# arclab-hku/ESVIO

Measured on AMD Instinct MI355X. Metric: Mevents/s through time-surface+detect+track @640x480, higher is better.
Workload: dtype f64 timestamps / u8 images / f32 LK sums in the reference build's order

## Files before the change

esvio_amd/csrc/fe_api.cpp:

```cpp
#include "fe_internal.h"

namespace {
typedef int (*nccl_allgather_fn)(const void*, void*, size_t, int , void* ,
                                 hipStream_t);
struct NcclId {
  char internal[128];
};
typedef int (*nccl_get_id_fn)(NcclId*);
typedef int (*nccl_init_rank_fn)(void** , int, NcclId, int);
typedef int (*nccl_destroy_fn)(void*);
void* rccl_lib() {
  static void* lib = []() -> void* {
    const char* names[] = {"librccl.so.1", "librccl.so"};
    for (const char* n : names)
      if (void* l = dlopen(n, RTLD_NOW | RTLD_NOLOAD | RTLD_GLOBAL)) return l;
    for (const char* n : names)
      if (void* l = dlopen(n, RTLD_NOW | RTLD_GLOBAL)) return l;
    return dlopen("/opt/rocm/lib/librccl.so.1", RTLD_NOW | RTLD_GLOBAL);
  }();
  return lib;
}
template <class F>
F rccl_sym(const char* name) {
  void* l = rccl_lib();
// ... 179 lines not shown
  if ((rc = c->d_rejected.alloc(c, 1))) return bail(rc);
  if ((rc = c->d_res.alloc(c, res_layout(Mc).total))) return bail(rc);
  c->dres = res_view(c->d_res, Mc, 0);
  c->dres.mask = nullptr;
  {
    uint8_t* z_spec = nullptr;
    const size_t bytes = kSpecBlocks * spec_layout(Mc).bytes;
    if ((rc = c->h_spec.alloc(c, bytes))) return bail(rc);
    if (hipHostGetDevicePointer((void**)&z_spec, c->h_spec, 0) != hipSuccess) return bail(ESVIO_FE_EHIP);
    std::memset(c->h_spec, 0, bytes);
    for (int b = 0; b < kSpecBlocks; b++) {
      c->hspec[b] = spec_view(c->h_spec, Mc, b);
      c->zspec[b] = spec_view(z_spec, Mc, b);
    }
  }
  if ((rc = c->d_chain.alloc(c, 2 * std::max<size_t>(M, 1)))) return bail(rc);
  if ((rc = c->d_lane_gate.alloc(c, 16))) return bail(rc);
  c->stage_threads = stager_threads_from_env();
  if (const char* v = getenv("ESVIO_FE_FAULT")) esvio_fe_debug_inject(c, atoi(v));
  if (const char* e = getenv("ESVIO_FE_STEREO_SPLIT")) c->stereo_split_env = atoi(e) != 0;
  c->chain_enabled = getenv("ESVIO_FE_NO_CHAIN") == nullptr;
  c->cam_split_enabled = getenv("ESVIO_FE_NO_CAMSPLIT") == nullptr;
  c->dedup_enabled = getenv("ESVIO_FE_NO_DEDUP") == nullptr && (cfg->max_cnt > 500 || getenv("ESVIO_FE_DEDUP") != nullptr);
  c->fuse_ts_pyr = getenv("ESVIO_FE_NO_FUSE") == nullptr;
  c->fast_lds = getenv("ESVIO_FE_FAST_LDS") != nullptr;
  if (const char* v = getenv("ESVIO_FE_CONVERT_PINNED_COPY")) c->cvt_pinned_copy = atoi(v) != 0 ? 1 : 0;
  c->select_one_wave = getenv("ESVIO_FE_SELECT_SERIAL") != nullptr;
  if (const char* v = getenv("ESVIO_FE_SAE_EV_MIN")) c->sae_ev_min = (size_t)strtoull(v, nullptr, 10);
  c->tiled = make_tile_geom(c->W, c->H, &c->tgeom) && getenv("ESVIO_FE_SAE_SORT") == nullptr;
  for (int i = 0; i < kRightSlots; i++)
    if ((rc = c->d_first[i].alloc(c, (size_t)c->P))) return bail(rc);
  for (int i = 0; i < kRightSlots; i++) {
    const size_t words = arc_bitmap_words(c->W, c->H);
    if ((rc = c->d_cmap[i].alloc(c, words))) return bail(rc);
    if ((rc = c->d_touched[i].alloc(c, arc_flag_bytes(c->W, c->H)))) return bail(rc);
    if (hipMemsetAsync(c->d_cmap[i], 0, words * 4, cur_stream(c)) != hipSuccess ||
        hipMemsetAsync(c->d_touched[i], 0, arc_flag_bytes(c->W, c->H), cur_stream(c)) != hipSuccess)
      return bail(ESVIO_FE_EHIP);
  }
  if ((rc = c->d_pub_slots.alloc(c, std::max<size_t>(M, 1)))) return bail(rc);
  if ((rc = c->d_pub_done.alloc(c, 1))) return bail(rc);
  if (hipMemsetAsync(c->d_lane_gate, 0, 64, cur_stream(c)) != hipSuccess ||
      hipMemsetAsync(c->d_chain, 0, std::max<size_t>(M, 1) * 16, cur_stream(c)) != hipSuccess ||
      hipMemsetAsync(c->d_pub_slots, 0, std::max<size_t>(M, 1) * 8, cur_stream(c)) != hipSuccess ||
      hipMemsetAsync(c->d_pub_done, 0, 8, cur_stream(c)) != hipSuccess)
    return bail(ESVIO_FE_EHIP);
  if ((rc = c->d_ptsD.alloc(c, M))) return bail(rc);
  if ((rc = c->d_sel_idx.alloc(c, M))) return bail(rc);
  if ((rc = c->d_mask_bits.alloc(c, (size_t)c->H * ((c->W + 31) / 32)))) return bail(rc);
  for (PyrStore& ps : c->pyr)
    if ((rc = pyr_alloc(c, ps, c->W, c->H, 3))) return bail(rc);
  if (cfg->median_blur_kernel_size > 0)
    for (PyrStore& ps : c->med_tmp)
      if ((rc = pyr_alloc(c, ps, c->W, c->H, 0))) return bail(rc);
  if (cfg->equalize) {
    for (auto& rb : c->raw)
      for (PyrStore& ps : rb)
        if ((rc = pyr_alloc(c, ps, c->W, c->H, 0))) return bail(rc);
// ... 1137 lines not shown
    return ESVIO_FE_EHIP;
  }
  return 0;
}

int esvio_fe_unregister_host_buffer(void* p) {
  if (!p) return ESVIO_FE_EINVAL;
  if (hipHostUnregister(p) != hipSuccess) {
    (void)hipGetLastError();
    return ESVIO_FE_EHIP;
  }
  return 0;
}

int esvio_fe_debug_inject(esvio_fe_handle c, int mask) {
  if (!c || mask < 0 || mask > 31) return ESVIO_FE_EINVAL;
  c->lim = esvio_fe_ctx::WaitLimits();
  c->lazy_late = (mask & ESVIO_FE_FAULT_LAZY_LATE) != 0;
  if (mask & ESVIO_FE_FAULT_TICKET) c->lim.ticket = 0;
  if (mask & ESVIO_FE_FAULT_LOOKBACK) c->lim.lookback = 0;
  if (mask & ESVIO_FE_FAULT_SPECULATIVE) c->lim.poll = 0;
  if (mask & ESVIO_FE_FAULT_CHAINED) c->lim.chain = 0;
  return 0;
}

int esvio_fe_debug_counters(esvio_fe_handle c, uint64_t out4[4]) {
  if (!c || !out4) return ESVIO_FE_EINVAL;
  out4[0] = c->n_spec_expired;
  out4[1] = c->n_chain_expired;
  out4[2] = c->tr_chain_launch;
  out4[3] = c->tr_chain_used;
  return 0;
}

int esvio_fe_plain_call_counters(esvio_fe_handle c, uint64_t out4[4]) {
  if (!c || !out4) return ESVIO_FE_EINVAL;
  out4[0] = c->n_plain_calls;
// ... 138 lines not shown
```

esvio_amd/csrc/fe_ctx.h:

```cpp
#pragma once
#include <hip/hip_runtime.h>

#include <algorithm>
#include <atomic>
#include <chrono>
#include <cmath>
#include <cstdarg>
#include <cstdio>
#include <cstdlib>
#include <cstring>
#include <dlfcn.h>
#include <map>
#include <string>
#include <utility>
#include <deque>
#include <vector>

#include "../../include/esvio_fe.h"
#include "../../include/esvio_fe_test.h"
#include "fe_host.h"
#include "fe_kernels.h"
#include "fe_layout.h"
#include "fe_mc.h"
#include "fe_res.h"
// ... 143 lines not shown
  bool x_deferred = false;
  std::deque<Batch> announced;
  std::deque<Inflight> inflight;
  bool cur_prefetched = false;
  EventStager* stager = nullptr;
  std::atomic<int> stage_pending{0};
  int cur_stage = -1;
  int stage_threads = 0;
  Launcher* launcher = nullptr;
  uint64_t lane_job[kPrefetchDepth] = {};
  int launch_err = 0;
  uint64_t lks_wait_job[2] = {};
  struct WaitLimits {
    uint32_t lookback = kSpinLookback, ticket = kSpinTicket;
    unsigned long long poll = kTicksPoll, chain = kTicksChain;
  } lim;
  bool lazy_late = false;
  uint64_t n_spec_expired = 0, n_chain_expired = 0;
  DevBuf<EventRec> d_evp[kPrefetchDepth];
  Event ev_lane_done[kPrefetchDepth], ev_lane_arc[kPrefetchDepth];
  PyrStore tmp_pyr[2];
  PyrStore med_tmp[2];
  PyrStore raw[kRightSlots][2];
  int raw_cur = 0;
  DevBuf<uint8_t> d_lut;
  DevBuf<int> d_minmax;
  DevBuf<uint8_t> d_res;
  ResView dres{};
  DevBuf<float2> d_ptsD;
  ResView pin[2] = {}, zpin[2] = {};
  SpecView hspec[kSpecBlocks] = {}, zspec[kSpecBlocks] = {};
  int res_set = 0;
  int lks_last = -1;
  PinBuf<uint8_t> h_spec;
  bool spec_valid = false;
  int spec_n = 0;
  DevBuf<unsigned long long> d_chain;
  DevBuf<uint32_t> d_lane_gate;
  uint32_t gate_seq = 0;
  int n_cu = 0;
  bool waits_fit_spec = true, waits_fit_chain = true;
  uint32_t chain_seq = 0;
  bool chain_enabled = true;
  bool cam_split_enabled = true;
  uint64_t n_plain_calls = 0, n_cam_split = 0, n_stereo_chained = 0;
  bool chain_valid = false;
  uint64_t chain_for = 0;
  bool chain_map_ok = false;
  std::vector<int> chain_map;
  uint64_t frame_no = 0;
  Event ev_chain_done;
  DevBuf<unsigned long long> d_pub_slots, d_pub_done;
// ... 212 lines not shown
```

esvio_amd/csrc/fe_kernels.h:

```cpp
#pragma once
#include <hip/hip_runtime.h>
#include <stdint.h>
#include <stdlib.h>

#include <vector>

namespace esvio {


struct __attribute__((aligned(16))) EventRec {
  uint16_t x, y;
  uint32_t sec, nsec;
  uint8_t pol;
  uint8_t pad[3];
};
static_assert(sizeof(EventRec) == 16, "event record must be 16 B");

constexpr int kPad = 24;
constexpr int kMaxLevels = 4;
constexpr int kLkWin = 21;
constexpr int kArcBlock = 256;
constexpr int kMaxDiscR = 63;

struct PyrDesc {
// ... 180 lines not shown
  PyrDesc N;
  const float2* prev_pts;
  const float2* init_pts;
  float2* next_pts;
  uint8_t* status;
  const int* n_ptr;
  int n_max;
  const unsigned long long* poll_slots = nullptr;
  const unsigned long long* poll_done = nullptr;
  uint32_t poll_seq = 0;
  int poll_from = 0;
  int* poll_err = nullptr;
  unsigned long long* chain_out = nullptr;
  const unsigned long long* chain_in = nullptr;
  uint32_t chain_seq = 0;
  unsigned long long poll_ticks = kTicksPoll, chain_ticks = kTicksChain;
  const uint32_t* gate_ptr = nullptr;
  uint32_t gate_val = 0;
  int max_level;
  int max_count;
  double eps2;
  int flags;
  int accum = 1;
};
void launch_lk(hipStream_t s, const LkArgs& f, const LkArgs* b, float2* back_pts,
               uint8_t* back_status);

struct ArcArgs {
  const EventRec* ev;
  uint32_t n;
// ... 122 lines not shown
```

esvio_amd/csrc/fe_kernels.hip:

```cpp
#include "fe_kernels.h"
#include "fe_mc.h"

#include <algorithm>
#include <cstdio>
#include <cstdlib>
#include <cstring>
#include <tuple>
#include <type_traits>

namespace esvio {

namespace {
template <typename... P, typename... A>
void launch_k(void (*kernel)(P...), dim3 grid, dim3 block, unsigned shmem, hipStream_t s, A... args) {
  static_assert(sizeof...(P) == sizeof...(A), "argument count");
  hipLaunchKernelGGL(kernel, grid, block, shmem, s, args...);
}
}

__device__ __forceinline__ int lane_id() { return threadIdx.x & 63; }

__device__ __forceinline__ double ev_time(uint32_t sec, uint32_t nsec) {
  return __dadd_rn((double)sec, __dmul_rn(1e-9, (double)nsec));
}
// ... 2018 lines not shown
__device__ __forceinline__ uint32_t mad_u24_regw(uint32_t oy, uint32_t ox) {
  uint32_t r;
  static_assert(kLkRegW <= 64, "inline constant");
  asm("v_mad_u32_u24 %0, %1, %2, %3" : "=v"(r) : "v"(oy), "n"(kLkRegW), "v"(ox));
  return r;
}
__device__ __forceinline__ int sdot2_zero(uint32_t a, uint32_t b) {
  int r;
  asm("v_dot2_i32_i16 %0, %1, %2, 0" : "=v"(r) : "v"(a), "v"(b));
  return r;
}
__device__ __forceinline__ int sdot2_seed(uint32_t a, uint32_t b, int seed) {
  int r;
  asm("v_dot2_i32_i16 %0, %1, %2, %3" : "=v"(r) : "v"(a), "v"(b), "s"(seed));
  return r;
}

template <int ACCUM>
__device__ __forceinline__ void lk_point(const LkCall& c, const float2 prev0, const float2 init,
                                         uint32_t* regJ, uint32_t term_base, float* acc_ta, const LkLaneF32* lnf, int lane,
                                         float2& np_out, int& st_out) {
  constexpr int WIN = kLkWin, NP = ACCUM == 2 ? 8 : 7, NPP = 4, NL = kMaxLevels;
  const float halfWin = (WIN - 1) * 0.5f;
  const int W_BITS = 14;
  const RedLane rl = red_lane(lane);
  const bool on = ACCUM == 2 || lane < 63;
  const int plane = ACCUM == 2 ? min(lane, 62) : lane;
  const int row = on ? plane / 3 : 0;
  const int x0 = on ? (plane - row * 3) * NP : 0;
  const int lane_bo = row * kLkRegW + x0;
// ... 297 lines not shown
          break;
        }
      }
      (void)restage;
    }
    if (st && L == 0) {
      const float fx = np.x - halfWin, fy = np.y - halfWin;
      const int ix = (int)floorf(fx), iy = (int)floorf(fy);
      if (ix < -WIN || ix >= cols || iy < -WIN || iy >= rows) st = 0;
    }
  }
  np_out = np;
  st_out = st;
}

struct LkKernelArgs {
  LkCall fwd;
  LkCall back;
  int have_back;
  const float2* prev_pts;
  const float2* init_pts;
  float2* next_pts;
  uint8_t* status;
  float2* back_pts;
  uint8_t* back_status;
  const int* n_ptr;
  int n_max;
  const unsigned long long* poll_slots;
  const unsigned long long* poll_done;
  uint32_t poll_seq;
  int poll_from;
  int* poll_err;
  unsigned long long* chain_out;
  const unsigned long long* chain_in;
  uint32_t chain_seq;
  unsigned long long poll_ticks, chain_ticks;
  const uint32_t* gate_ptr;
  uint32_t gate_val;
};

__device__ __forceinline__ void chain_publish(const LkKernelArgs& a, int pt, int lane, float2 p, int alive) {
  if (!a.chain_out || lane != 0) return;
  const unsigned long long hi = (unsigned long long)((a.chain_seq << 2) | (uint32_t)(alive ? 1 : 0)) << 32;
  __hip_atomic_store(&a.chain_out[2 * pt], hi | __float_as_uint(p.x), __ATOMIC_RELAXED, __HIP_MEMORY_SCOPE_AGENT);
  __hip_atomic_store(&a.chain_out[2 * pt + 1], hi | __float_as_uint(p.y), __ATOMIC_RELAXED,
                     __HIP_MEMORY_SCOPE_AGENT);
}

template <int ACCUM>
__device__ __forceinline__ void lk_kernel_body(const LkKernelArgs& a, uint32_t (*regJ_s)[kLkRegStore], uint32_t acc_t,
                                               float* acc_ta, const LkLaneF32* lnf) {
  const int wave = threadIdx.x >> 6, lane = lane_id();
  const int pt = blockIdx.x * kLkWaves + wave;
  const int n = a.n_ptr ? *a.n_ptr : a.n_max;
// ... 59 lines not shown
      __builtin_amdgcn_s_sleep(16);
    }
    prev0 = make_float2((float)(uint32_t)(v & 0xffffu), (float)(uint32_t)((v >> 16) & 0xffffu));
  } else {
    prev0 = a.prev_pts[pt];
  }
  const float2 init = (a.fwd.flags & 4) ? a.init_pts[pt] : make_float2(0.f, 0.f);
  float2 np;
  int st;
  lk_point<ACCUM>(a.fwd, prev0, init, regJ_s[wave], acc_t, acc_ta, lnf, lane, np, st);
  chain_publish(a, pt, lane, np, st);
  if (lane == 0) {
    a.next_pts[pt] = np;
    a.status[pt] = (uint8_t)st;
  }
  if (a.have_back) {
    float2 bp;
    int bs;
    lk_point<ACCUM>(a.back, np, prev0, regJ_s[wave], acc_t, acc_ta, lnf, lane, bp, bs);
    if (lane == 0) {
      a.back_pts[pt] = bp;
      a.back_status[pt] = (uint8_t)bs;
    }
  }
}

__global__ __launch_bounds__(64 * kLkWaves) void k_lk(LkKernelArgs a) {
  __shared__ __attribute__((aligned(16))) uint32_t regJ_s[kLkWaves][kLkRegStore];
  lk_kernel_body<1>(a, regJ_s, 0u, nullptr, nullptr);
}
__global__ __launch_bounds__(64 * kLkWaves) void k_lk_f32(LkKernelArgs a) {
  __shared__ __attribute__((aligned(16))) uint32_t regJ_s[kLkWaves][kLkRegStore];
  __shared__ __attribute__((aligned(16))) int term_all[kLkWaves][kF32TermWords];
  __shared__ __attribute__((aligned(16))) float term_a[kLkWaves][kLkTermWordsA];
  const int wave = threadIdx.x >> 6, lane = threadIdx.x & 63;
  for (int i = lane; i < kF32TermWords; i += 64) term_all[wave][i] = 0;
  {
    const int l = lane < 63 ? lane : 62, t = l / kLkWin, rw = l - t * kLkWin;
// ... 38 lines not shown
  a.back_status = back_status;
  a.n_ptr = f.n_ptr;
  a.n_max = f.n_max;
  a.poll_slots = f.poll_slots;
  a.poll_done = f.poll_done;
  a.poll_seq = f.poll_seq;
  a.poll_from = f.poll_from;
  a.poll_err = f.poll_err;
  a.chain_out = f.chain_out;
  a.chain_in = f.chain_in;
  a.chain_seq = f.chain_seq;
  a.poll_ticks = f.poll_ticks;
  a.chain_ticks = f.chain_ticks;
  a.gate_ptr = f.gate_ptr;
  a.gate_val = f.gate_val;
  if (f.accum == 2)
    launch_k(k_lk_f32, dim3((a.n_max + kLkWaves - 1) / kLkWaves), dim3(64 * kLkWaves), 0, s, a);
  else
    launch_k(k_lk, dim3((a.n_max + kLkWaves - 1) / kLkWaves), dim3(64 * kLkWaves), 0, s, a);
}

__constant__ int8_t c_small[16][2] = {{0, 3},  {1, 3},   {2, 2},   {3, 1},  {3, 0},  {3, -1},
                                      {2, -2}, {1, -3},  {0, -3},  {-1, -3}, {-2, -2}, {-3, -1},
                                      {-3, 0}, {-3, 1},  {-2, 2},  {-1, 3}};
__constant__ int8_t c_large[20][2] = {{0, 4},   {1, 4},   {2, 3},   {3, 2},  {4, 1},  {4, 0},  {4, -1},
                                      {3, -2},  {2, -3},  {1, -4},  {0, -4}, {-1, -4}, {-2, -3}, {-3, -2},
                                      {-4, -1}, {-4, 0},  {-4, 1},  {-3, 2}, {-2, 3},  {-1, 4}};

template <int N>
struct RingRanks {
// ... 1331 lines not shown
```

esvio_amd/csrc/fe_layout.h:

```cpp
#pragma once
#include <cstddef>
#include <cstdint>

namespace esvio {
namespace fe {

struct P2f {
  float x, y;
};

struct LkOut {
  P2f *fwd, *back;
  uint8_t *st_fwd, *st_back;
};

inline size_t layout_points(int max_cnt) { return max_cnt > 1 ? (size_t)max_cnt : 1; }
inline size_t round_up(size_t v, size_t to) { return (v + to - 1) / to * to; }

struct ResLayout {
  size_t B1[2], C1[2], SA1[2], SB1[2], A[2], CNT, NEW, B2, C2, SA2, SB2, total;
  size_t mask;
};
inline ResLayout res_layout(int max_cnt) {
  const size_t M = layout_points(max_cnt), stM = round_up(M, 64);
// ... 54 lines not shown
  v.counts = (int*)(b + L.CNT);
  v.mask = (uint32_t*)(b + L.mask);
  return v;
}

struct SpecView {
  LkOut out;
  int* expired;
};
inline SpecView spec_view(uint8_t* b, int max_cnt, int block) {
  const SpecLayout L = spec_layout(max_cnt);
  b += (size_t)block * L.bytes;
  return SpecView{LkOut{(P2f*)(b + L.B), (P2f*)(b + L.C), b + L.SA, b + L.SB}, (int*)(b + L.expired)};
}

}
}
```

esvio_amd/csrc/fe_stages.cpp:

```cpp
#include "fe_internal.h"

namespace esvio {
namespace fe {


int ensure_event_capacity(esvio_fe_ctx* c, size_t n) { return c->d_ev.grow(c, n); }

static int grow_sort_buffers(esvio_fe_ctx* c, size_t cap) {
  c->sort_cap = 0;
  for (int i = 0; i < 2; i++) {
    c->keys[i].release();
    c->vals[i].release();
  }
  for (int i = 0; i < 2; i++) {
    if (int rc = c->keys[i].alloc(c, cap)) return rc;
    if (int rc = c->vals[i].alloc(c, cap)) return rc;
  }
  if (int rc = c->sae_marks.alloc(c, cap)) return rc;
  c->sort_cap = cap;
  return 0;
}

int ensure_sort_capacity(esvio_fe_ctx* c, size_t n) {
  if (n > c->sort_cap)
// ... 399 lines not shown
  LkArgs fa = f;
  fa.accum = c->cfg.lk_accum;
  launch_lk(cur_stream(c), fa, b, back_pts, back_status);
}

LkPair lk_pair(const PyrDesc& P, const PyrDesc& N, const P2f* src, const int* n_ptr, int n_max, LkPairKind kind,
               const LkOut& out) {
  const bool t = kind == kLkTemporal;
  return LkPair{make_lk(P, N, (const float2*)src, nullptr, (float2*)out.fwd, out.st_fwd, n_ptr, n_max, 3, 30, 0.01, 0),
                make_lk(N, P, nullptr, nullptr, nullptr, nullptr, n_ptr, n_max, t ? 1 : 3, 30, 0.01,
                        t ? ESVIO_FE_LK_USE_INITIAL_FLOW : 0),
                out};
}

void run_lk_pair(esvio_fe_ctx* c, const LkPair& p) {
  run_lk(c, p.f, c->cfg.flow_back ? &p.b : nullptr, (float2*)p.out.back, p.out.st_back);
}

static int image_stage_slot(esvio_fe_ctx* c, size_t bytes, size_t* off) {
  constexpr int kSlots = 4;
  if (!c->d_img || c->d_img.cap < kSlots * bytes) {
    HIPCHK(c, hipStreamSynchronize(cur_stream(c)));
    c->d_img.release();
    if (int rc = c->h_img.alloc(c, kSlots * bytes)) return rc;
    if (int rc = c->d_img.alloc(c, kSlots * bytes)) return rc;
  }
  *off = (size_t)(c->img_stage_next++ % kSlots) * (c->d_img.cap / kSlots);
  return 0;
}

int copy_level0_in(esvio_fe_ctx* c, const PyrDesc& d, const uint8_t* in) {
// ... 298 lines not shown
```

esvio_amd/csrc/fe_track.cpp:

```cpp
#include "fe_internal.h"

#include <sched.h>
#include <sys/resource.h>

#include <atomic>
#include <condition_variable>
#include <mutex>
#include <thread>

namespace esvio {
namespace fe {

struct PrefetchJob {
  Inflight b;
  bool wait_planes = false;
  int lks_wait = -1;
};

static int prefetch_issue(esvio_fe_ctx* c, const PrefetchJob& j) {
  const Inflight& b = j.b;
  StreamScope on_prefetch_stream(c->stream2);
  if (j.wait_planes) HIPCHK(c, hipStreamWaitEvent(c->stream2, c->ev_planes_free, 0));
  if (j.lks_wait >= 0) HIPCHK(c, hipStreamWaitEvent(c->stream2, c->ev_lks_done[j.lks_wait], 0));
  const EventRec *dL = b.dL, *dR = b.dR;
// ... 221 lines not shown
    } else {
      rc = prefetch_issue(c, job);
      if (!rc && b.stage < 0 && b.space == ESVIO_FE_HOST) {
        b.dL = c->d_evp[b.lane];
        b.dR = c->d_evp[b.lane] + b.nL;
      }
    }
    if (rc) break;
    c->inflight.push_back(b);
    c->announced.pop_front();
    if (only_first) break;
  }
  return rc;
}

static uint32_t next_chain_seq(esvio_fe_ctx* c) {
  c->chain_seq = (c->chain_seq + 1) & 0x3fffffffu;
  if (!c->chain_seq) c->chain_seq = 1;
  return c->chain_seq;
}

int enqueue_spec_temporal(esvio_fe_ctx* c, const Inflight& nxt ,
                          int n_kept, bool with_new) {
  if (int rc = launcher_wait_lane(c, nxt.lane)) return rc;
  HIPCHK(c, hipStreamWaitEvent(c->stream3, c->ev_lane_done[nxt.lane], 0));
  const PyrDesc& P = c->pyr[c->slot_curL].d;
  const PyrDesc& N = c->pyr[nxt.slotL].d;
  const int n_max = with_new ? (int)layout_points(c->cfg.max_cnt) : n_kept;
  LkPair sp = lk_pair(P, N, c->zpin[0].news, nullptr, n_max, kLkTemporal, c->zspec[0].out);
  if (with_new) {
    sp.f.poll_slots = c->d_pub_slots;
    sp.f.poll_done = c->d_pub_done;
    sp.f.poll_seq = c->pub_seq;
    sp.f.poll_from = n_kept;
    sp.f.poll_err = c->zspec[0].expired;
    sp.f.poll_ticks = c->lim.poll;
  }
  const Inflight* nxt2 = nullptr;
  if (c->chain_enabled && c->waits_fit_chain && !nxt.pub && c->inflight.size() >= 2 && c->inflight[0].lane == nxt.lane &&
      !c->chain_valid)
    nxt2 = &c->inflight[1];
  if (nxt2) {
    sp.f.chain_out = c->d_chain;
    sp.f.chain_seq = next_chain_seq(c);
  }
  {
    StreamScope on_spec_stream(c->stream3);
    run_lk_pair(c, sp);
  }
  HIPCHK(c, hipEventRecord(c->ev_spec_done, c->stream3));
  c->spec_valid = true;
  if (nxt2) {
    const bool gated = c->launcher && nxt2->gate != 0;
    if (!gated)
      if (int rc = launcher_wait_lane(c, nxt2->lane)) return rc;
    HIPCHK(c, hipStreamWaitEvent(c->stream4, c->ev_lane_done[nxt.lane], 0));
    if (!gated) HIPCHK(c, hipStreamWaitEvent(c->stream4, c->ev_lane_done[nxt2->lane], 0));
    const PyrDesc& N2 = c->pyr[nxt2->slotL].d;
    LkPair ch = lk_pair(N, N2, nullptr, nullptr, n_max, kLkTemporal, c->zspec[1].out);
    ch.f.chain_in = c->d_chain;
    ch.f.chain_seq = c->chain_seq;
    ch.f.chain_ticks = c->lim.chain;
    ch.f.poll_err = c->zspec[1].expired;
    if (gated) {
      ch.f.gate_ptr = c->d_lane_gate + nxt2->lane;
      ch.f.gate_val = nxt2->gate;
    }
    {
      StreamScope on_chain_stream(c->stream4);
      run_lk_pair(c, ch);
    }
    HIPCHK(c, hipEventRecord(c->ev_chain_done, c->stream4));
    c->chain_valid = true;
    c->tr_chain_launch++;
    c->chain_for = c->frame_no + 2;
    c->chain_map_ok = false;
  }
  return 0;
// ... 115 lines not shown
  const esvio_fe_motion* motion;
  const int M;
  ResView pin{}, zpin{};
  const EventRec *dL = nullptr, *dR = nullptr;
  bool first = false;
  bool arc_done = false, arc_prefetched = false, arc_marked_main = false;
  int arc_lane = 0;
  bool main_reads_events = false;
  bool main_reads_planes = false;
  bool have_next = false, had_announced = false;
  Inflight next_b;
  bool early_done = false, defer_late = false;
  bool use_spec = false, use_chain = false, chain_covers_next = false;
  bool will_spec = false, detect = false;
  bool plain = false, arc_side = false, stereo_chained = false;
  bool split_right = false;
  int set_st = 0;
  std::vector<int> surv_src;
  int n_surv = 0, n_kept = 0;
  clk::time_point tp;

  TrackCall(esvio_fe_ctx* ctx, double t, const esvio_fe_event* l, size_t nl, const esvio_fe_event* r, size_t nr,
            int sp, bool pub, const esvio_fe_motion* mo)
      : c(ctx), time(t), left(l), right(r), nL(nl), nR(nr), space(sp), PUB_THIS_FRAME(pub), motion(mo),
        M(ctx->cfg.max_cnt) {}

  void lap(int i) {
    const auto now = clk::now();
    const double ms = std::chrono::duration<double, std::milli>(now - tp).count();
    c->lat.cur_phase[i] += ms;
// ... 265 lines not shown
            g_ptsC[j] = r.back[k];
            g_stA[j] = r.st_fwd[k];
            g_stB[j] = r.st_back[k];
          }
          t = LkOut{g_ptsB.data(), g_ptsC.data(), g_stA.data(), g_stB.data()};
        }
      }
      if (!spec_ok) {
        std::memcpy(pin.A, c->prev_pts.data(), (size_t)n * 8);
        LkPair lk = lk_pair(prevL, curL, zpin.A, nullptr, n, kLkTemporal, zpin.s1);
        stereo_chained = plain && c->chain_enabled && c->waits_fit_chain;
        if (stereo_chained) {
          c->n_stereo_chained++;
          lk.f.chain_out = c->d_chain;
          lk.f.chain_seq = next_chain_seq(c);
        }
        run_lk_pair(c, lk);
        if (stereo_chained) {
          const PyrDesc& curR = c->pyr[c->slot_curR].d;
          set_st = c->res_set ^ 1;
          LkPair st = lk_pair(curL, curR, nullptr, nullptr, n, kLkStereo, c->zpin[set_st].s1);
          st.f.chain_in = c->d_chain;
          st.f.chain_seq = c->chain_seq;
          st.f.chain_ticks = c->lim.chain;
          st.f.poll_err = c->zspec[1].expired;
          StreamScope on_stereo_stream(stereo_stream(c));
          HIPCHK(c, hipStreamWaitEvent(stereo_stream(c), c->ev_imgs_ready, 0));
          run_lk_pair(c, st);
          if (int rc = record_lks_done(c, c->res_set)) return rc;
        }
        if (int rc = early_work()) return rc;
        if (int rc = exchange_flush(c)) return rc;
        pre_lift();
        lap(1);
        HIPCHK(c, sync_main(c));
        lap(2);
        t = pin.s1;
      }
      std::vector<uint8_t> status(t.st_fwd, t.st_fwd + n);
      c->cur_pts.resize(n);
      std::memcpy(c->cur_pts.data(), t.fwd, (size_t)n * 8);
      if (cfg.flow_back) {
        const P2f* reverse_pts = t.back;
        for (int i = 0; i < n; i++) {
          if (status[i] && t.st_back[i] && pt_distance(c->prev_pts[i], reverse_pts[i]) <= 0.5)
            status[i] = 1;
          else
            status[i] = 0;
        }
      }
      for (int i = 0; i < n; i++)
        if (status[i] && !in_border_event(c, c->cur_pts[i])) status[i] = 0;
      if (chain_covers_next) {
        if (use_spec && spec_ok) {
          c->chain_map.clear();
          for (int i = 0; i < n; i++)
            if (status[i]) c->chain_map.push_back(i);
          c->chain_map_ok = true;
        } else if (int rc = cancel_chain(c)) {
          return rc;
        }
      }
      if (stereo_chained) {
        surv_src.clear();
        for (int i = 0; i < n; i++)
          if (status[i]) surv_src.push_back(i);
      }
      if (c->pre_lift_valid) {
        reduce_vector(c->pre_lx, status);
        reduce_vector(c->pre_ly, status);
      }
      reduce_vector(c->prev_pts, status);
      reduce_vector(c->cur_pts, status);
      reduce_vector(c->ids, status);
      reduce_vector(c->track_cnt, status);
    } else if (chain_covers_next) {
      if (int rc = cancel_chain(c)) return rc;
    }
// ... 152 lines not shown
    const bool lazy = c->lazy_new && detect;
    const bool defer_right = c->lazy_new && !PUB_THIS_FRAME;
    bool pending_later = false;
    if (defer_right && c->pend.active && !c->pend_right.active) {
      pending_later = c->lazy_late || !event_over(c->ev_lknew_done);
    }
    if (!pending_later)
      if (int rc = finalize_lazy(c)) return rc;
    tail_lap(1);
    if (defer_right) {
    } else {
      if (!lazy) HIPCHK(c, sync_main(c));
      if (n_surv || stereo_chained) HIPCHK(c, sync_event(c->ev_lks_done[c->res_set]));
      if (stereo_chained) {
        int* wait_expired = c->hspec[1].expired;
        if (*wait_expired != 0) {
          *wait_expired = 0;
          c->n_chain_expired++;
          const int n = (int)surv_src.size() ? surv_src.back() + 1 : 0;
          if (n) {
            const PyrDesc& curL = c->pyr[c->slot_curL].d;
            const PyrDesc& curR = c->pyr[c->slot_curR].d;
            StreamScope on_stereo_stream(stereo_stream(c));
            run_lk_pair(c, lk_pair(curL, curR, zpin.s1.fwd, nullptr, n, kLkStereo, c->zpin[set_st].s1));
            HIPCHK(c, hipStreamSynchronize(stereo_stream(c)));
          }
        }
      }
    }
    lap(6);
    tt = clk::now();
// ... 150 lines not shown
```

esvio_amd/frontend.py:

```python
import ctypes as C
import os

import numpy as np

from . import build as _build

_HERE = os.path.dirname(os.path.abspath(__file__))
HOST, DEVICE = 0, 1
LK_USE_INITIAL_FLOW = 4


class FrontendError(RuntimeError):
    pass


class Camera(C.Structure):
    _fields_ = [(n, C.c_double) for n in ("fx", "fy", "cx", "cy", "k1", "k2", "p1", "p2")]


class Config(C.Structure):
    _fields_ = [
        ("width", C.c_int32), ("height", C.c_int32),
        ("decay_ms", C.c_double),
        ("ignore_polarity", C.c_int32), ("median_blur_kernel_size", C.c_int32),
# ... 55 lines not shown
    "esvio_fe_convert_events", "esvio_fe_create",
    "esvio_fe_create_sae", "esvio_fe_create_sae_stereo", "esvio_fe_create_sae_stereo_mc", "esvio_fe_destroy",
    "esvio_fe_exchange_begin", "esvio_fe_exchange_end", "esvio_fe_exchange_tracks", "esvio_fe_export_image",
    "esvio_fe_fast_corners", "esvio_fe_features_to_track", "esvio_fe_find_fundamental_mat", "esvio_fe_finish", "esvio_fe_get_sae",
    "esvio_fe_get_time_surface", "esvio_fe_good_features_to_track", "esvio_fe_import_image", "esvio_fe_is_corner",
    "esvio_fe_last_error", "esvio_fe_mem_alloc", "esvio_fe_mem_free", "esvio_fe_mem_upload",
    "esvio_fe_pack_track_records", "esvio_fe_register_host_buffer", "esvio_fe_reserve", "esvio_fe_reset",
    "esvio_fe_sae_plane_doubles", "esvio_fe_sae_slice_apply", "esvio_fe_sae_slice_commit",
    "esvio_fe_sae_slice_last", "esvio_fe_sae_to_time_surface", "esvio_fe_set_auto_exchange",
    "esvio_fe_set_host_threads", "esvio_fe_set_launch_thread", "esvio_fe_set_lazy_new_stereo",
    "esvio_fe_set_next_batch", "esvio_fe_set_next_batch_mc", "esvio_fe_track_event", "esvio_fe_track_event_fields",
    "esvio_fe_track_event_mc",
    "esvio_fe_track_image", "esvio_fe_unregister_host_buffer", "esvio_fe_version",
]
TEST_SYMBOLS = [
    "esvio_fe_build_pyramid", "esvio_fe_debug_counters", "esvio_fe_debug_inject", "esvio_fe_device_memory",
    "esvio_fe_find_fundamental_mat_held", "esvio_fe_find_fundamental_mat_idle", "esvio_fe_find_fundamental_mat_mt",
    "esvio_fe_get_kernel_stats", "esvio_fe_host_hypot", "esvio_fe_host_nullspace", "esvio_fe_host_stage_copy",
    "esvio_fe_host_stage_pack", "esvio_fe_staging_counters",
    "esvio_fe_kernel_count", "esvio_fe_kernel_name", "esvio_fe_latency_phase_name", "esvio_fe_latency_recent",
    "esvio_fe_latency_stats", "esvio_fe_lift_projective", "esvio_fe_plain_call_counters", "esvio_fe_ransac_stats",
    "esvio_fe_ransac_tail", "esvio_fe_reset_kernel_stats", "esvio_fe_set_profiling", "esvio_fe_set_sae",
    "esvio_fe_stream",
]

LATENCY_PHASES = 16


class LatencyCall(C.Structure):
    _fields_ = [("call", C.c_uint64), ("published", C.c_int32), ("reserved", C.c_int32), ("begin_ms", C.c_double),
                ("ms", C.c_double), ("phase_ms", C.c_double * 16)]
# ... 45 lines not shown
    L.esvio_fe_lift_projective.argtypes = [C.POINTER(Camera), d, d, vp]
    L.esvio_fe_track_event.argtypes = [vp, d, vp, sz, vp, sz, i, i, C.POINTER(Tracks)]
    L.esvio_fe_track_event_mc.argtypes = [vp, d, vp, sz, vp, sz, i, i, C.POINTER(Motion),
                                          C.POINTER(Tracks)]
    L.esvio_fe_create_sae_stereo_mc.argtypes = [vp, vp, sz, vp, sz, i, C.POINTER(Motion),
                                                C.POINTER(C.c_uint64)]
    L.esvio_fe_set_next_batch.argtypes = [vp, d, vp, sz, vp, sz, i, i]
    L.esvio_fe_set_next_batch_mc.argtypes = [vp, d, vp, sz, vp, sz, i, i, C.POINTER(Motion)]
    L.esvio_fe_mem_alloc.argtypes = [i, sz, vp]
    L.esvio_fe_mem_free.argtypes = [i, vp]
    L.esvio_fe_mem_upload.argtypes = [vp, vp, sz]
    L.esvio_fe_register_host_buffer.argtypes = [vp, sz]
    L.esvio_fe_unregister_host_buffer.argtypes = [vp]
    L.esvio_fe_debug_inject.argtypes = [vp, i]
    L.esvio_fe_debug_counters.argtypes = [vp, vp]
    L.esvio_fe_plain_call_counters.argtypes = [vp, vp]
    L.esvio_fe_good_features_to_track.argtypes = [vp, vp, i, d, d, vp, vp, vp, vp]
    L.esvio_fe_track_image.argtypes = [vp, d, vp, vp, i, vp]
    L.esvio_fe_pack_track_records.argtypes = [vp, vp, vp]
    L.esvio_fe_set_lazy_new_stereo.argtypes = [vp, i]
    L.esvio_fe_set_host_threads.argtypes = [vp, i]
    L.esvio_fe_ransac_stats.argtypes = [vp, i]
    L.esvio_fe_host_hypot.argtypes = [vp, vp, i, vp]
    L.esvio_fe_host_stage_copy.argtypes = [vp, vp, C.c_size_t]
    L.esvio_fe_host_nullspace.argtypes = [vp, i, i, vp, C.POINTER(C.c_int32)]
    L.esvio_fe_find_fundamental_mat_mt.argtypes = [vp, vp, i, d, d, i, vp, C.POINTER(C.c_int32)]
    L.esvio_fe_finish.argtypes = [vp, vp]
    L.esvio_fe_get_time_surface.argtypes = [vp, i, vp]
    L.esvio_fe_export_image.argtypes = [vp, i, vp, i]
    L.esvio_fe_import_image.argtypes = [vp, i, vp, i]
# ... 57 lines not shown
    c.device = device
    cams = kw.get("cams")
    if cams is None:
        cams = [dict(fx=0.9 * W, fy=0.9 * W, cx=W / 2.0, cy=H / 2.0, k1=-0.05, k2=0.01, p1=1e-4,
                     p2=-2e-4)] * 2
    for k in range(2):
        for n in ("fx", "fy", "cx", "cy", "k1", "k2", "p1", "p2"):
            setattr(c.cam[k], n, float(cams[k][n]))
    return c


def _p(a):
    return a.ctypes.data_as(C.c_void_p) if a is not None else None


FAULT_TICKET, FAULT_LOOKBACK, FAULT_SPECULATIVE, FAULT_CHAINED, FAULT_LAZY_LATE = 1, 2, 4, 8, 16


def _events_arg(ev):
    if isinstance(ev, tuple):
        return C.c_void_p(ev[0]), int(ev[1]), DEVICE, None
    ev = np.ascontiguousarray(ev)
    if ev.dtype.itemsize != 16:
        raise ValueError("events must be 16-byte records (esvio_amd.events.EVENT_DTYPE)")
    return _p(ev), ev.shape[0], HOST, ev


class _Handle:
    def __init__(self, cfg):
        self.L = load_library()
        self.cfg = cfg
# ... 240 lines not shown
            out.append((int(o.call), bool(o.published), o.begin_ms, o.ms,
                        {names[k]: o.phase_ms[k] for k in range(LATENCY_PHASES) if o.phase_ms[k] > 0.0005}))
        return out

    def debug_inject(self, mask):
        self._hd.check(self._hd.L.esvio_fe_debug_inject(self._hd.h, int(mask)))

    def staging_counters(self):
        out = (C.c_uint64 * 4)()
        self._hd.check(self._hd.L.esvio_fe_staging_counters(self._hd.h, out))
        return dict(batches=out[0], bytes=out[1], chunks_packed=out[2], chunks_raw=out[3])

    def debug_counters(self):
        out = (C.c_uint64 * 4)()
        self._hd.check(self._hd.L.esvio_fe_debug_counters(self._hd.h, out))
        return dict(spec_redone=out[0], chain_redone=out[1], chain_launched=out[2], chain_used=out[3])

    def plain_call_counters(self):
        out = (C.c_uint64 * 4)()
        self._hd.check(self._hd.L.esvio_fe_plain_call_counters(self._hd.h, out))
        return dict(plain_calls=out[0], split_by_camera=out[1], stereo_chained=out[2], chained_redone=out[3])

    def comm_init(self, unique_id, rank, world):
        buf = (C.c_uint8 * 128).from_buffer_copy(bytes(unique_id))
        self._hd.check(self._hd.L.esvio_fe_comm_init(self._hd.h, buf, int(rank), int(world)))
        self._x_world = int(world)

    def set_auto_exchange(self, on=True):
        self._hd.check(self._hd.L.esvio_fe_set_auto_exchange(self._hd.h, int(bool(on))))

    def exchange_begin(self):
# ... 322 lines not shown
```

Measured before the change: 2825.

## Abandon chained LK back-tracks for points the producer already knows are dropped

When a producer LK kernel's backward check shows a point will be rejected (back status zero or round-trip distance over a bound), it publishes a per-point drop word in a new third section of the chain buffer. The chained consumer kernel reads that word and skips its own backward LK for the point, marking it dead and counting abandonments. Points whose forward status is already zero also skip the backward pass. The host re-checks the drop rule against its final keep mask and falls back to the redo path on a mismatch. This trades extra atomics, a larger chain buffer and extra host verification for less wasted backward tracking.

```diff
diff --git a/esvio_amd/csrc/fe_api.cpp b/esvio_amd/csrc/fe_api.cpp
--- a/esvio_amd/csrc/fe_api.cpp
+++ b/esvio_amd/csrc/fe_api.cpp
@@ -217,12 +217,13 @@
       c->zspec[b] = spec_view(z_spec, Mc, b);
     }
   }
-  if ((rc = c->d_chain.alloc(c, 2 * std::max<size_t>(M, 1)))) return bail(rc);
+  if ((rc = c->d_chain.alloc(c, 3 * std::max<size_t>(M, 1)))) return bail(rc);
   if ((rc = c->d_lane_gate.alloc(c, 16))) return bail(rc);
   c->stage_threads = stager_threads_from_env();
   if (const char* v = getenv("ESVIO_FE_FAULT")) esvio_fe_debug_inject(c, atoi(v));
   if (const char* e = getenv("ESVIO_FE_STEREO_SPLIT")) c->stereo_split_env = atoi(e) != 0;
   c->chain_enabled = getenv("ESVIO_FE_NO_CHAIN") == nullptr;
+  c->abandon_enabled = getenv("ESVIO_FE_NO_ABANDON") == nullptr;
   c->cam_split_enabled = getenv("ESVIO_FE_NO_CAMSPLIT") == nullptr;
   c->dedup_enabled = getenv("ESVIO_FE_NO_DEDUP") == nullptr && (cfg->max_cnt > 500 || getenv("ESVIO_FE_DEDUP") != nullptr);
   c->fuse_ts_pyr = getenv("ESVIO_FE_NO_FUSE") == nullptr;
@@ -244,7 +245,7 @@
   if ((rc = c->d_pub_slots.alloc(c, std::max<size_t>(M, 1)))) return bail(rc);
   if ((rc = c->d_pub_done.alloc(c, 1))) return bail(rc);
   if (hipMemsetAsync(c->d_lane_gate, 0, 64, cur_stream(c)) != hipSuccess ||
-      hipMemsetAsync(c->d_chain, 0, std::max<size_t>(M, 1) * 16, cur_stream(c)) != hipSuccess ||
+      hipMemsetAsync(c->d_chain, 0, std::max<size_t>(M, 1) * 24, cur_stream(c)) != hipSuccess ||
       hipMemsetAsync(c->d_pub_slots, 0, std::max<size_t>(M, 1) * 8, cur_stream(c)) != hipSuccess ||
       hipMemsetAsync(c->d_pub_done, 0, 8, cur_stream(c)) != hipSuccess)
     return bail(ESVIO_FE_EHIP);
@@ -1412,13 +1413,26 @@
 }
 
 int esvio_fe_debug_inject(esvio_fe_handle c, int mask) {
-  if (!c || mask < 0 || mask > 31) return ESVIO_FE_EINVAL;
+  if (!c || mask < 0 || mask > 63) return ESVIO_FE_EINVAL;
   c->lim = esvio_fe_ctx::WaitLimits();
   c->lazy_late = (mask & ESVIO_FE_FAULT_LAZY_LATE) != 0;
   if (mask & ESVIO_FE_FAULT_TICKET) c->lim.ticket = 0;
   if (mask & ESVIO_FE_FAULT_LOOKBACK) c->lim.lookback = 0;
   if (mask & ESVIO_FE_FAULT_SPECULATIVE) c->lim.poll = 0;
   if (mask & ESVIO_FE_FAULT_CHAINED) c->lim.chain = 0;
+  if (mask & ESVIO_FE_FAULT_ALL_DROPPED) c->lim.drop_d2 = -1.f;
+  return 0;
+}
+
+int esvio_fe_abandon_counters(esvio_fe_handle c, uint64_t out4[4]) {
+  if (!c || !out4) return ESVIO_FE_EINVAL;
+  uint32_t n = 0;
+  HIPCHK(c, hipSetDevice(c->dev));
+  HIPCHK(c, hipMemcpy(&n, c->dres.counts + 8, 4, hipMemcpyDeviceToHost));
+  out4[0] = n;
+  out4[1] = c->n_abandon_mismatch;
+  out4[2] = c->n_drop_launches;
+  out4[3] = c->abandon_enabled ? 1 : 0;
   return 0;
 }
 
diff --git a/esvio_amd/csrc/fe_ctx.h b/esvio_amd/csrc/fe_ctx.h
--- a/esvio_amd/csrc/fe_ctx.h
+++ b/esvio_amd/csrc/fe_ctx.h
@@ -181,6 +181,7 @@
   struct WaitLimits {
     uint32_t lookback = kSpinLookback, ticket = kSpinTicket;
     unsigned long long poll = kTicksPoll, chain = kTicksChain;
+    float drop_d2 = kDropDist2;
   } lim;
   bool lazy_late = false;
   uint64_t n_spec_expired = 0, n_chain_expired = 0;
@@ -203,6 +204,9 @@
   bool spec_valid = false;
   int spec_n = 0;
   DevBuf<unsigned long long> d_chain;
+  bool abandon_enabled = true;
+  float chain_drop_d2 = 0.f;
+  uint64_t n_abandon_mismatch = 0, n_drop_launches = 0;
   DevBuf<uint32_t> d_lane_gate;
   uint32_t gate_seq = 0;
   int n_cu = 0;
diff --git a/esvio_amd/csrc/fe_kernels.h b/esvio_amd/csrc/fe_kernels.h
--- a/esvio_amd/csrc/fe_kernels.h
+++ b/esvio_amd/csrc/fe_kernels.h
@@ -218,6 +218,11 @@
   unsigned long long* chain_out = nullptr;
   const unsigned long long* chain_in = nullptr;
   uint32_t chain_seq = 0;
+  unsigned long long* drop_out = nullptr;
+  const unsigned long long* drop_in = nullptr;
+  float drop_d2 = 0.f;
+  uint32_t* abandoned = nullptr;
+  bool skip_dead = false;
   unsigned long long poll_ticks = kTicksPoll, chain_ticks = kTicksChain;
   const uint32_t* gate_ptr = nullptr;
   uint32_t gate_val = 0;
diff --git a/esvio_amd/csrc/fe_kernels.hip b/esvio_amd/csrc/fe_kernels.hip
--- a/esvio_amd/csrc/fe_kernels.hip
+++ b/esvio_amd/csrc/fe_kernels.hip
@@ -1,4 +1,5 @@
 #include "fe_kernels.h"
+#include "fe_layout.h"
 #include "fe_mc.h"
 
 #include <algorithm>
@@ -2056,6 +2057,46 @@
   int r;
   asm("v_dot2_i32_i16 %0, %1, %2, %3" : "=v"(r) : "v"(a), "v"(b), "s"(seed));
   return r;
+}
+
+struct LkKernelArgs {
+  LkCall fwd;
+  LkCall back;
+  int have_back;
+  const float2* prev_pts;
+  const float2* init_pts;
+  float2* next_pts;
+  uint8_t* status;
+  float2* back_pts;
+  uint8_t* back_status;
+  const int* n_ptr;
+  int n_max;
+  const unsigned long long* poll_slots;
+  const unsigned long long* poll_done;
+  uint32_t poll_seq;
+  int poll_from;
+  int* poll_err;
+  unsigned long long* chain_out;
+  const unsigned long long* chain_in;
+  uint32_t chain_seq;
+  unsigned long long poll_ticks, chain_ticks;
+  const uint32_t* gate_ptr;
+  uint32_t gate_val;
+  unsigned long long* drop_out;
+  const unsigned long long* drop_in;
+  float drop_d2;
+  uint32_t* abandoned;
+  int skip_dead;
+};
+
+__device__ __forceinline__ bool lk_dropped() {
+  const LkKernelArgs* ka = (const LkKernelArgs*)__builtin_amdgcn_kernarg_segment_ptr();
+  asm volatile("" : "+s"(ka));
+  const unsigned long long* w = ka->drop_in;
+  if (!w) return false;
+  const int pt = blockIdx.x * kLkWaves + __builtin_amdgcn_readfirstlane(threadIdx.x >> 6);
+  const uint32_t v = __hip_atomic_load((const uint32_t*)(w + pt) + 1, __ATOMIC_RELAXED, __HIP_MEMORY_SCOPE_AGENT);
+  return (uint32_t)__builtin_amdgcn_readfirstlane((int)v) == ((ka->chain_seq << 2) | 1u);
 }
 
 template <int ACCUM>
@@ -2383,30 +2424,6 @@
   st_out = st;
 }
 
-struct LkKernelArgs {
-  LkCall fwd;
-  LkCall back;
-  int have_back;
-  const float2* prev_pts;
-  const float2* init_pts;
-  float2* next_pts;
-  uint8_t* status;
-  float2* back_pts;
-  uint8_t* back_status;
-  const int* n_ptr;
-  int n_max;
-  const unsigned long long* poll_slots;
-  const unsigned long long* poll_done;
-  uint32_t poll_seq;
-  int poll_from;
-  int* poll_err;
-  unsigned long long* chain_out;
-  const unsigned long long* chain_in;
-  uint32_t chain_seq;
-  unsigned long long poll_ticks, chain_ticks;
-  const uint32_t* gate_ptr;
-  uint32_t gate_val;
-};
 
 __device__ __forceinline__ void chain_publish(const LkKernelArgs& a, int pt, int lane, float2 p, int alive) {
   if (!a.chain_out || lane != 0) return;
@@ -2496,14 +2513,31 @@
     a.next_pts[pt] = np;
     a.status[pt] = (uint8_t)st;
   }
-  if (a.have_back) {
-    float2 bp;
-    int bs;
-    lk_point<ACCUM>(a.back, np, prev0, regJ_s[wave], acc_t, acc_ta, lnf, lane, bp, bs);
+  if (!a.have_back) return;
+  if (a.skip_dead && !st) {
     if (lane == 0) {
-      a.back_pts[pt] = bp;
-      a.back_status[pt] = (uint8_t)bs;
-    }
+      a.back_pts[pt] = np;
+      a.back_status[pt] = 0;
+    }
+    return;
+  }
+  if (lk_dropped()) {
+    if (lane == 0) {
+      a.status[pt] = 0;
+      a.back_status[pt] = 0;
+      if (a.abandoned) __hip_atomic_fetch_add(a.abandoned, 1u, __ATOMIC_RELAXED, __HIP_MEMORY_SCOPE_AGENT);
+    }
+    return;
+  }
+  float2 bp;
+  int bs;
+  lk_point<ACCUM>(a.back, np, prev0, regJ_s[wave], acc_t, acc_ta, lnf, lane, bp, bs);
+  if (lane == 0) {
+    a.back_pts[pt] = bp;
+    a.back_status[pt] = (uint8_t)bs;
+    if (a.drop_out && fe::surely_dropped(bs, prev0.x, prev0.y, bp.x, bp.y, a.drop_d2))
+      __hip_atomic_store(&a.drop_out[pt], (unsigned long long)((a.chain_seq << 2) | 1u) << 32, __ATOMIC_RELAXED,
+                         __HIP_MEMORY_SCOPE_AGENT);
   }
 }
 
@@ -2572,6 +2606,11 @@
   a.chain_ticks = f.chain_ticks;
   a.gate_ptr = f.gate_ptr;
   a.gate_val = f.gate_val;
+  a.drop_out = f.drop_out;
+  a.drop_in = f.drop_in;
+  a.drop_d2 = f.drop_d2;
+  a.abandoned = f.abandoned;
+  a.skip_dead = f.skip_dead ? 1 : 0;
   if (f.accum == 2)
     launch_k(k_lk_f32, dim3((a.n_max + kLkWaves - 1) / kLkWaves), dim3(64 * kLkWaves), 0, s, a);
   else
diff --git a/esvio_amd/csrc/fe_layout.h b/esvio_amd/csrc/fe_layout.h
--- a/esvio_amd/csrc/fe_layout.h
+++ b/esvio_amd/csrc/fe_layout.h
@@ -92,5 +92,15 @@
   return SpecView{LkOut{(P2f*)(b + L.B), (P2f*)(b + L.C), b + L.SA, b + L.SB}, (int*)(b + L.expired)};
 }
 
+constexpr float kDropDist2 = 0.2625f;
+#if defined(__HIPCC__) || defined(__CUDACC__)
+__host__ __device__
+#endif
+inline bool surely_dropped(int back_status, float px, float py, float bx, float by, float bound) {
+  if (!back_status) return true;
+  const float dx = px - bx, dy = py - by;
+  return dx * dx + dy * dy > bound;
+}
+
 }
 }
diff --git a/esvio_amd/csrc/fe_stages.cpp b/esvio_amd/csrc/fe_stages.cpp
--- a/esvio_amd/csrc/fe_stages.cpp
+++ b/esvio_amd/csrc/fe_stages.cpp
@@ -437,7 +437,9 @@
 }
 
 void run_lk_pair(esvio_fe_ctx* c, const LkPair& p) {
-  run_lk(c, p.f, c->cfg.flow_back ? &p.b : nullptr, (float2*)p.out.back, p.out.st_back);
+  LkArgs f = p.f;
+  f.skip_dead = c->abandon_enabled;
+  run_lk(c, f, c->cfg.flow_back ? &p.b : nullptr, (float2*)p.out.back, p.out.st_back);
 }
 
 static int image_stage_slot(esvio_fe_ctx* c, size_t bytes, size_t* off) {
diff --git a/esvio_amd/csrc/fe_track.cpp b/esvio_amd/csrc/fe_track.cpp
--- a/esvio_amd/csrc/fe_track.cpp
+++ b/esvio_amd/csrc/fe_track.cpp
@@ -259,6 +259,27 @@
   return rc;
 }
 
+static void drop_word_out(esvio_fe_ctx* c, LkArgs& producer) {
+  if (!c->abandon_enabled || !c->cfg.flow_back) return;
+  producer.drop_out = c->d_chain + 2 * layout_points(c->cfg.max_cnt);
+  producer.drop_d2 = c->chain_drop_d2 = c->lim.drop_d2;
+  c->n_drop_launches++;
+}
+static void drop_word_in(esvio_fe_ctx* c, LkArgs& consumer) {
+  if (!c->abandon_enabled || !c->cfg.flow_back) return;
+  consumer.drop_in = c->d_chain + 2 * layout_points(c->cfg.max_cnt);
+  consumer.abandoned = (uint32_t*)(c->dres.counts + 8);
+}
+
+static bool drop_rule_mismatch(esvio_fe_ctx* c, const std::vector<uint8_t>& kept, const LkOut& t, const P2f* prev, int n) {
+  if (!c->abandon_enabled || !c->cfg.flow_back) return false;
+  bool bad = false;
+  for (int i = 0; i < n; i++)
+    if (kept[i] && surely_dropped(t.st_back[i], prev[i].x, prev[i].y, t.back[i].x, t.back[i].y, c->chain_drop_d2)) bad = true;
+  if (bad) c->n_abandon_mismatch++;
+  return bad;
+}
+
 static uint32_t next_chain_seq(esvio_fe_ctx* c) {
   c->chain_seq = (c->chain_seq + 1) & 0x3fffffffu;
   if (!c->chain_seq) c->chain_seq = 1;
@@ -288,6 +309,7 @@
   if (nxt2) {
     sp.f.chain_out = c->d_chain;
     sp.f.chain_seq = next_chain_seq(c);
+    drop_word_out(c, sp.f);
   }
   {
     StreamScope on_spec_stream(c->stream3);
@@ -307,6 +329,7 @@
     ch.f.chain_seq = c->chain_seq;
     ch.f.chain_ticks = c->lim.chain;
     ch.f.poll_err = c->zspec[1].expired;
+    drop_word_in(c, ch.f);
     if (gated) {
       ch.f.gate_ptr = c->d_lane_gate + nxt2->lane;
       ch.f.gate_val = nxt2->gate;
@@ -452,6 +475,7 @@
   bool use_spec = false, use_chain = false, chain_covers_next = false;
   bool will_spec = false, detect = false;
   bool plain = false, arc_side = false, stereo_chained = false;
+  bool stereo_mismatch = false;
   bool split_right = false;
   int set_st = 0;
   std::vector<int> surv_src;
@@ -747,6 +771,7 @@
           c->n_stereo_chained++;
           lk.f.chain_out = c->d_chain;
           lk.f.chain_seq = next_chain_seq(c);
+          drop_word_out(c, lk.f);
         }
         run_lk_pair(c, lk);
         if (stereo_chained) {
@@ -757,6 +782,7 @@
           st.f.chain_seq = c->chain_seq;
           st.f.chain_ticks = c->lim.chain;
           st.f.poll_err = c->zspec[1].expired;
+          drop_word_in(c, st.f);
           StreamScope on_stereo_stream(stereo_stream(c));
           HIPCHK(c, hipStreamWaitEvent(stereo_stream(c), c->ev_imgs_ready, 0));
           run_lk_pair(c, st);
@@ -785,7 +811,7 @@
       for (int i = 0; i < n; i++)
         if (status[i] && !in_border_event(c, c->cur_pts[i])) status[i] = 0;
       if (chain_covers_next) {
-        if (use_spec && spec_ok) {
+        if (use_spec && spec_ok && !drop_rule_mismatch(c, status, t, c->prev_pts.data(), n)) {
           c->chain_map.clear();
           for (int i = 0; i < n; i++)
             if (status[i]) c->chain_map.push_back(i);
@@ -795,6 +821,7 @@
         }
       }
       if (stereo_chained) {
+        stereo_mismatch = drop_rule_mismatch(c, status, t, c->prev_pts.data(), n);
         surv_src.clear();
         for (int i = 0; i < n; i++)
           if (status[i]) surv_src.push_back(i);
@@ -977,7 +1004,7 @@
       if (n_surv || stereo_chained) HIPCHK(c, sync_event(c->ev_lks_done[c->res_set]));
       if (stereo_chained) {
         int* wait_expired = c->hspec[1].expired;
-        if (*wait_expired != 0) {
+        if (*wait_expired != 0 || stereo_mismatch) {
           *wait_expired = 0;
           c->n_chain_expired++;
           const int n = (int)surv_src.size() ? surv_src.back() + 1 : 0;
diff --git a/esvio_amd/frontend.py b/esvio_amd/frontend.py
--- a/esvio_amd/frontend.py
+++ b/esvio_amd/frontend.py
@@ -93,7 +93,7 @@
     "esvio_fe_track_image", "esvio_fe_unregister_host_buffer", "esvio_fe_version",
 ]
 TEST_SYMBOLS = [
-    "esvio_fe_build_pyramid", "esvio_fe_debug_counters", "esvio_fe_debug_inject", "esvio_fe_device_memory",
+    "esvio_fe_abandon_counters", "esvio_fe_build_pyramid", "esvio_fe_debug_counters", "esvio_fe_debug_inject", "esvio_fe_device_memory",
     "esvio_fe_find_fundamental_mat_held", "esvio_fe_find_fundamental_mat_idle", "esvio_fe_find_fundamental_mat_mt",
     "esvio_fe_get_kernel_stats", "esvio_fe_host_hypot", "esvio_fe_host_nullspace", "esvio_fe_host_stage_copy",
     "esvio_fe_host_stage_pack", "esvio_fe_staging_counters",
@@ -169,6 +169,7 @@
     L.esvio_fe_unregister_host_buffer.argtypes = [vp]
     L.esvio_fe_debug_inject.argtypes = [vp, i]
     L.esvio_fe_debug_counters.argtypes = [vp, vp]
+    L.esvio_fe_abandon_counters.argtypes = [vp, vp]
     L.esvio_fe_plain_call_counters.argtypes = [vp, vp]
     L.esvio_fe_good_features_to_track.argtypes = [vp, vp, i, d, d, vp, vp, vp, vp]
     L.esvio_fe_track_image.argtypes = [vp, d, vp, vp, i, vp]
@@ -256,7 +257,7 @@
     return a.ctypes.data_as(C.c_void_p) if a is not None else None
 
 
-FAULT_TICKET, FAULT_LOOKBACK, FAULT_SPECULATIVE, FAULT_CHAINED, FAULT_LAZY_LATE = 1, 2, 4, 8, 16
+FAULT_TICKET, FAULT_LOOKBACK, FAULT_SPECULATIVE, FAULT_CHAINED, FAULT_LAZY_LATE, FAULT_ALL_DROPPED = 1, 2, 4, 8, 16, 32
 
 
 def _events_arg(ev):
@@ -527,7 +528,10 @@
     def debug_counters(self):
         out = (C.c_uint64 * 4)()
         self._hd.check(self._hd.L.esvio_fe_debug_counters(self._hd.h, out))
-        return dict(spec_redone=out[0], chain_redone=out[1], chain_launched=out[2], chain_used=out[3])
+        ab = (C.c_uint64 * 4)()
+        self._hd.check(self._hd.L.esvio_fe_abandon_counters(self._hd.h, ab))
+        return dict(spec_redone=out[0], chain_redone=out[1], chain_launched=out[2], chain_used=out[3],
+                    chain_abandoned=ab[0], chain_abandon_mismatch=ab[1], drop_word_launches=ab[2], abandon_on=ab[3])
 
     def plain_call_counters(self):
         out = (C.c_uint64 * 4)()
```

Result: slower. 2622 (-7.2%).
